# kasvii/GATOR

Measured on AMD Instinct MI355X. Metric: meshes/sec (B=256, J=17) GATOR forward, higher is better.
Workload: dtype f32; 1 GPU; B=256 synthetic Human3.6M 17-joint poses per GPU, GAT+MDR forward fp32; batch_per_gpu=256, global_batch=256, num_joint=17, impl=fused, parallelism=dp1, mode=gather

## Files before the change

### gator_amd/csrc/fused_api.hip

```cpp
#include <hip/hip_runtime.h>

#include <algorithm>
#include <cmath>
#include <cstdlib>
#include <type_traits>
#include <vector>

#include "fused_state.h"
#include "x3_common.h"

namespace gator {
namespace {

static void graph_slot_free(FusedState::GraphSlot& g) {
    if (g.exec) (void)hipGraphExecDestroy((hipGraphExec_t)g.exec);
    if (g.graph) (void)hipGraphDestroy((hipGraph_t)g.graph);
    g.exec = g.graph = nullptr;
}
static void graphs_clear(FusedState* f) {
    for (auto& g : f->graphs) graph_slot_free(g);
    f->graphs.clear();
}
struct WsScope {
    FusedState* f; FusedWs* prev;
    WsScope(FusedState* f_, int i) : f(f_), prev(f_->ws) { f->ws = &f->sets[i]; }
    ~WsScope() { f->ws = prev; }
};

int fused_ensure_ws(gator_ctx* c, int B) {
    FusedState* f = c->fused;
    FusedWs& w = *f->ws;
    if (w.base && B <= w.cap) return GATOR_OK;
    if (w.base) {
        GATOR_HIP_CHECK(hipDeviceSynchronize());
        graphs_clear(f);
    }
    const int cap = B, MT = (cap + 31) / 32, J = c->J;
    const size_t tiles = (size_t)cap * kVT * 2 * kTile;
    size_t n = 0;
    auto layout = [&](float* block) {
        n = 0;
        auto region = [&](auto*& member, size_t floats) {
            if (block) member = reinterpret_cast<std::remove_reference_t<decltype(member)>>(block + n);
            n += (floats + 63) & ~(size_t)63;
        };
        region(w.vcp, (size_t)MT * 3 * kCB * kTile); region(w.vc, (size_t)cap * kV * 3);
        region(w.vf, 3 * tiles); region(w.q, 9 * tiles / 2); region(w.k, 9 * tiles / 2); region(w.v, 9 * tiles / 2);
        region(w.jkv, (size_t)cap * 12 * kTile); region(w.hf, (size_t)cap * kV * 32); region(w.lbf, (size_t)cap * kV * kE);
        region(w.feat, (size_t)cap * J * kC); region(w.vcp3, std::max(upsample_x3_vcp_elems(cap), upsample_x2_vcp_elems(cap)) / 2);
        region(w.lpart, gat_tail_part_floats(cap, J)); region(w.mdr_ctr, mdr_ctr_words(cap)); region(w.hpart, (size_t)cap * kVT * 128);
    };
    layout(nullptr);
    GATOR_TRY(w.base.alloc(n * sizeof(float)));
    GATOR_HIP_CHECK(hipMemset(w.base, 0, n * sizeof(float)));
    GATOR_HIP_CHECK(hipDeviceSynchronize());
    w.cap = cap;
    layout(w.base);
    return GATOR_OK;
}

std::vector<float> d2h(const float* p, size_t n) {
    std::vector<float> v(n);
    (void)hipMemcpy(v.data(), p, n * sizeof(float), hipMemcpyDeviceToHost);
    return v;
}

template <class F>
void fill_tile(float* dst, F tab) {
    for (int g = 0; g < 4; ++g)
        for (int lane = 0; lane < 64; ++lane)
            for (int j = 0; j < 4; ++j) dst[(g * 64 + lane) * 4 + j] = tab(lane & 31, 8 * g + 4 * (lane >> 5) + j);
}

int read_fused_options(const gator_ctx* c, FusedOptions* o) {
    auto flag = [](const char* name, bool dflt) { const char* e = getenv(name); return e ? atoi(e) != 0 : dflt; };
    auto num = [](const char* name, int dflt) { const char* e = getenv(name); return e ? atoi(e) : dflt; };
    auto set = [](const char* name) { return getenv(name) != nullptr; };
    const bool exact = c->arithmetic == GATOR_ARITH_EXACT_SPLIT;
    o->gat_x3 = flag("GATOR_GAT_X3", true);
    o->gat8 = o->gat_x3 && flag("GATOR_GAT8", true);
    o->gat8_h4 = !exact && flag("GATOR_GAT8_H4", true);
    o->gat8_lobyte = o->gat8 && o->gat8_h4 && flag("GATOR_GAT8_LOBYTE", true);
    o->gat_tiled_h4 = !exact && flag("GATOR_GAT_TILED_H4", true);
    o->gat_tiled = num("GATOR_GAT_TILED", -1);
    if (const int m = num("GATOR_GAT_TILED_MIN_BATCH", 0); m > 0) o->gat_tiled_min_batch = m;
    o->mdr_x3 = exact ? 1 : num("GATOR_MDR_X3", 2);
    o->up_x3 = exact ? 1 : num("GATOR_UPSAMPLE_X3", 2);
    if (c->parts & GATOR_PART_MDR) {
        if (o->up_x3 < 0 || o->up_x3 > 2) return fail(GATOR_EINVAL, "GATOR_UPSAMPLE_X3 must be 0, 1 or 2");
        if (o->mdr_x3 < 0 || o->mdr_x3 > 2) return fail(GATOR_EINVAL, "GATOR_MDR_X3 must be 0, 1 or 2");
    }
    o->gat8_tail = o->gat8 && o->gat8_h4 && o->mdr_x3 == 2 && flag("GATOR_GAT8_TAIL", true);
    o->mdr_persist = set("GATOR_MDR_PERSIST") ? flag("GATOR_MDR_PERSIST", false) : -1;
    o->mdr_persist_chunk = num("GATOR_MDR_PERSIST_CHUNK", 0);
    o->mdr_persist_grid = num("GATOR_MDR_PERSIST_GRID", 0);
    o->mdr_head_partials = flag("GATOR_MDR_HEAD_PARTIALS", true);
    o->c3_mdr = o->mdr_x3 == 2 && flag("GATOR_C3_MDR", true);
    o->c3_encoder = o->gat8 && o->gat8_h4 && o->gat_tiled_h4 && flag("GATOR_C3_ENCODER", true);
    o->c3_up_w1 = flag("GATOR_C3_UPSAMPLE_W1", true);
    o->c3_up_bf16 = o->up_x3 != 2 || flag("GATOR_C3_UPSAMPLE_BF16", false);
    o->c3_guard = flag("GATOR_C3_GUARD", true);
    o->graph = flag("GATOR_GRAPH", false);
    o->subbatch_streams = num("GATOR_SUBBATCH_STREAMS", 0);
#ifdef GATOR_DIAG
    o->gat8_dbg = num("GATOR_GAT8_DBG", 0);
    o->gat_stamps = set("GATOR_GAT_STAMPS");
    o->mdr_cut = num("GATOR_MDR_CUT", 0);
    o->mdr_stamps = set("GATOR_MDR_STAMPS");
    o->mdr_solo = set("GATOR_MDR_SOLO");
    o->mdr_ends = set("GATOR_MDR_ENDS");
#endif
    return GATOR_OK;
}

static double sym_eig_max(std::vector<double>& A, int n) {
    for (int sweep = 0; sweep < 64; ++sweep) {
        double off = 0, all = 0;
        for (int p = 0; p < n; ++p)
            for (int q = 0; q < n; ++q) { all += A[p * n + q] * A[p * n + q]; if (q > p) off += A[p * n + q] * A[p * n + q]; }
        if (!(off > 1e-30 * all)) break;
        for (int p = 0; p < n; ++p)
            for (int q = p + 1; q < n; ++q) {
                const double apq = A[p * n + q];
                if (apq == 0) continue;
                const double th = (A[q * n + q] - A[p * n + p]) / (2 * apq);
                const double t = (th >= 0 ? 1.0 : -1.0) / (std::fabs(th) + std::sqrt(th * th + 1));
                const double cs = 1 / std::sqrt(t * t + 1), sn = t * cs;
                for (int k = 0; k < n; ++k) {
                    const double kp = A[k * n + p], kq = A[k * n + q];
                    A[k * n + p] = cs * kp - sn * kq; A[k * n + q] = sn * kp + cs * kq;
                }
                for (int k = 0; k < n; ++k) {
                    const double pk = A[p * n + k], qk = A[q * n + k];
                    A[p * n + k] = cs * pk - sn * qk; A[q * n + k] = sn * pk + cs * qk;
                }
            }
    }
    double m = 0;
    for (int i = 0; i < n; ++i) m = std::max(m, A[i * n + i]);
    return m;
}

float c3_logit_bound(const Weights& w) {
    double worst = 0;
    for (int li = 0; li < 3; ++li) {
        const MdrLayerW& r = w.lay[li];
        const std::vector<float> wq = d2h(r.sa_w[0], 64 * 64), wk = d2h(r.sa_w[1], 64 * 64), bq = d2h(r.sa_b[0], 64), bk = d2h(r.sa_b[1], 64),
                                 a2 = d2h(r.a2, 64), b2 = d2h(r.b2, 64);
        double amax = 0, bn = 0;
        for (int i = 0; i < 64; ++i) { amax = std::max(amax, (double)std::fabs(a2[i])); bn += (double)b2[i] * b2[i]; }
        const double xn = amax * std::sqrt(63.0) + std::sqrt(bn);
        auto head_norm = [&](const std::vector<float>& W, const std::vector<float>& bias, int hd) {
            std::vector<double> G(32 * 32);
            double bb = 0;
            for (int i = 0; i < 32; ++i) {
                bb += (double)bias[32 * hd + i] * bias[32 * hd + i];
                for (int j = 0; j < 32; ++j) {
                    double acc = 0;
                    for (int k = 0; k < 64; ++k) acc += (double)W[(32 * hd + i) * 64 + k] * (double)W[(32 * hd + j) * 64 + k];
                    G[i * 32 + j] = acc;
                }
            }
            return std::sqrt(std::max(sym_eig_max(G, 32), 0.0)) * xn + std::sqrt(bb);
        };
        for (int hd = 0; hd < 2; ++hd)
            worst = std::max(worst, head_norm(wq, bq, hd) * head_norm(wk, bk, hd) / std::sqrt(32.0) * 1.4426950408889634);
    }
    return (float)worst;
}

struct PackItem { const float* src; int64_t wsn, wsk; int N, K; const float** dst; };
template <size_t n>
int pack_linears(const PackItem (&items)[n], float*& p, void* stream) {
    for (const PackItem& it : items) {
        GATOR_TRY(fused_pack_linear(it.src, it.wsn, it.wsk, it.N, it.K, p, stream));
        *it.dst = p;
        p += (size_t)nblk32(it.N) * nblk32(it.K) * kTile;
    }
    return GATOR_OK;
}

int fused_create_gat(gator_ctx* c, FusedState* f, void* stream) {
    const Weights& w = c->w;
    const int J = c->J;
    const size_t blk_tiles = 48 + 16 + 16 + 16 + 16 + 4 + 20 + 64 + 64 + 4 + 4 + 1 + 1;
    const size_t total = (kDepth * blk_tiles + 8 + 2 + 8 + 4 + 12) * kTile;
    GATOR_TRY(f->gbuf.alloc(total * sizeof(float)));
    float* p = f->gbuf;
    auto take = [&](size_t tiles) { float* r = p; p += tiles * kTile; return r; };
    std::vector<float> host;
    auto upload = [&](const std::vector<float>& v) -> const float* {
        float* d = take(v.size() / kTile);
        (void)hipMemcpy(d, v.data(), v.size() * sizeof(float), hipMemcpyHostToDevice);
        return d;
    };
    const std::vector<float> adiag = d2h(c->adj_diag, (size_t)kDepth * J), aoff = d2h(c->adj_off, (size_t)kDepth * J * J),
                             m1 = d2h(c->mask1, (size_t)J * J), m2 = d2h(c->mask2, (size_t)J * J), hb = d2h(c->hop_bias, (size_t)kH * J * J);
    for (int i = 0; i < kDepth; ++i) {
        const GatBlockW& r = w.blk[i];
        GatBlockPk& q = f->gblk[i];
        const PackItem items[] = {
            {r.qkv_w, 128, 1, 384, 128, &q.qkv}, {r.proj_w, 128, 1, 128, 128, &q.proj},
            {r.gcn_W, 1, 128, 128, 128, &q.w0}, {r.gcn_W + 128 * 128, 1, 128, 128, 128, &q.w1},
            {r.xl0_w, 128, 1, 128, 128, &q.lin0}, {r.xl1_w, 128, 1, 16, 128, &q.lin1}, {r.xlb_w, 144, 1, 128, 144, &q.back},
            {r.fc1_w, 128, 1, 512, 128, &q.fc1}, {r.fc2_w, 512, 1, 128, 512, &q.fc2}};
        GATOR_TRY(pack_linears(items, p, stream));
        const std::vector<float> M = d2h(r.gcn_M, (size_t)J * kC), b1 = d2h(r.xl1_b, 16);
        std::vector<float> mc(4 * kTile), md(4 * kTile);
        for (int nb = 0; nb < 4; ++nb) {
            for (int g = 0; g < 4; ++g)
                for (int lane = 0; lane < 64; ++lane)
                    for (int j = 0; j < 4; ++j) {
                        const int tok = 8 * g + 4 * (lane >> 5) + j, n = 32 * nb + (lane & 31);
                        mc[((nb * 4 + g) * 64 + lane) * 4 + j] = tok < J ? M[(size_t)tok * kC + n] : 0.f;
                    }
            fill_tile(md.data() + (size_t)nb * kTile, [&](int t, int ch) { return t < J ? adiag[i * J + t] * M[(size_t)t * kC + 32 * nb + ch] : 0.f; });
        }
        q.mc = upload(mc);
        q.mdT = upload(md);
        std::vector<float> t1(kTile), t2(kTile);
        fill_tile(t1.data(), [&](int t, int j) { return (t < J && j < J) ? aoff[((size_t)i * J + t) * J + j] : 0.f; });
        q.aoffT = upload(t1);
        fill_tile(t2.data(), [&](int t, int ch) {
            if (t >= J || ch >= 16) return 0.f;
            float deg = 0.f;
            for (int j = 0; j < J; ++j) deg += m2[(size_t)t * J + j];
            return deg * b1[ch];
        });
        q.f1b = upload(t2);
    }
    if (f->opt.gat_x3) {
        const int64_t ntiles = (p - f->gblk[0].qkv) / kTile;
        GATOR_TRY(f->gxbuf.alloc((size_t)ntiles * kTileX3 * sizeof(float)));
        int rc = fused_repack_x3(f->gblk[0].qkv, f->gxbuf, ntiles, stream);
        if (rc) return rc;
        if (f->opt.gat_tiled_h4) {
            float left = 0.f;
            GATOR_TRY(f->gxbuf_h3.alloc((size_t)ntiles * kTileX3 * sizeof(float)));
            rc = fused_repack_h3(f->gblk[0].qkv, f->gxbuf_h3, ntiles, &f->gat_tiled_wshift, &left, stream, (int64_t)blk_tiles, 264);
            if (rc == GATOR_OK && left > 1e-7f) rc = fail(GATOR_EUNSUPPORTED, "GAT weights span more than fp16 x 3 planes hold exactly: use GATOR_GAT_TILED_H4=0");
            if (rc) return rc;
        }
        if (f->opt.gat8) {
            rc = gat8_build_stream(f, stream);
            if (rc) return rc;
        }
    }
    std::vector<float> bt(8 * kTile), mt(kTile);
    for (int hd = 0; hd < kH; ++hd)
        fill_tile(bt.data() + (size_t)hd * kTile, [&](int t, int j) { return (t < J && j < J) ? hb[((size_t)hd * J + t) * J + j] : 0.f; });
    f->g_biasT = upload(bt);
    fill_tile(mt.data(), [&](int t, int j) { return (t < J && j < J) ? m1[(size_t)t * J + j] : 0.f; });
    f->g_m1T = upload(mt);
    fill_tile(mt.data(), [&](int t, int j) { return (t < J && j < J) ? m2[(size_t)t * J + j] : 0.f; });
    f->g_m2T = upload(mt);
    {
        std::vector<float> vv((size_t)kDepth * 2048);
        for (int i = 0; i < kDepth; ++i) {
            const GatBlockW& r = w.blk[i];
            const struct { const float* p; int n; } parts[] = {{r.n1w, 128}, {r.n1b, 128}, {r.qkv_b, 384}, {r.proj_b, 128}, {r.gcn_bias, 128},
                                                               {r.xl0_b, 128}, {r.xlb_b, 128}, {r.n2w, 128}, {r.n2b, 128}, {r.fc1_b, 512}, {r.fc2_b, 128}};
            size_t off = (size_t)i * 2048;
            for (auto& pt : parts) {
                const std::vector<float> h = d2h(pt.p, pt.n);
                std::copy(h.begin(), h.end(), vv.begin() + off);
                off += pt.n;
            }
        }
        f->g_vecs = upload(vv);
    }
    {
        float* dst = take(8);
        int rc = fused_pack_linear(w.gl3_W, 64, 1, 128, 64, dst, stream);
        if (rc) return rc;
        f->g_gl3 = dst;
        const std::vector<float> pe = d2h(c->pos_embed, (size_t)J * kC);
        std::vector<float> pt(4 * kTile);
        for (int kb = 0; kb < 4; ++kb)
            fill_tile(pt.data() + (size_t)kb * kTile, [&](int t, int ch) { return t < J ? pe[(size_t)t * kC + 32 * kb + ch] : 0.f; });
        f->g_posT = upload(pt);
    }
    {
        int rc = gat_prepare_device();
        if (rc == GATOR_OK) rc = gat_tiled_prepare_device();
        if (rc == GATOR_OK) rc = gat8_prepare_device();
        if (rc) return rc;
        hipDeviceProp_t prop;
        if (hipGetDeviceProperties(&prop, c->device) == hipSuccess && prop.multiProcessorCount > 0) f->n_cu = prop.multiProcessorCount;
    }
    GATOR_HIP_CHECK(hipStreamSynchronize((hipStream_t)stream));
    GATOR_HIP_CHECK(hipGetLastError());
    return GATOR_OK;
}

}

int fused_create(gator_ctx* c, void* stream) {
    if (c->impl == GATOR_IMPL_BASIC) return GATOR_OK;
    FusedState* f = new FusedState();
    c->fused = f;
    int rc = read_fused_options(c, &f->opt);
    if (rc) return rc;
    f->gat_tiled = f->opt.gat_tiled;
    f->graph_replay = f->opt.graph;
    const Weights& w = c->w;
    if (c->parts & GATOR_PART_GAT) {
        rc = fused_create_gat(c, f, stream);
        if (rc) return rc;
    }
    if (!(c->parts & GATOR_PART_MDR)) return GATOR_OK;
    if (f->opt.c3_mdr) {
        f->c3_logit_bound = c3_logit_bound(w);
        if (f->opt.c3_guard && !(f->c3_logit_bound <= 1024.0f)) f->opt.c3_mdr = f->opt.c3_encoder = false;
    }
    const size_t n_up = f->opt.up_x3 == 0 ? (size_t)3 * kOB * kCB * kTile : 0, n_layer = (size_t)64 * kTile;
    const size_t total = n_up + 3 * n_layer + 24 * kTile + 64 + (size_t)kVT * 2 * kTile + 3 * 64 + 1024;
    GATOR_TRY(f->wbuf.alloc(total * sizeof(float)));
    float* p = f->wbuf;
    auto take = [&](size_t k) { float* r = p; p += k; return r; };
    float* up = take(n_up);
    if (f->opt.up_x3 == 2) {
        GATOR_TRY(f->up_w2.alloc(upsample_x2_weight_elems() * 2));
        int rc = pack_upsample_x2(w.up_w, f->up_w2, &f->up_w2_unscale, stream);
        if (rc == GATOR_OK) rc = upsample_x2_prepare_device();
        if (rc) return rc;
    } else if (f->opt.up_x3 == 1) {
        GATOR_TRY(f->up_w3.alloc(upsample_x3_weight_elems() * 2));
        int rc = pack_upsample_x3(w.up_w, f->up_w3, stream);
        if (rc) return rc;
    } else {
        for (int tap = 0; tap < 3; ++tap) {
            int rc = fused_pack_linear(w.up_w + tap, (int64_t)kV * 3, 3, kNV, kV, up + (size_t)tap * kOB * kCB * kTile, stream);
            if (rc) return rc;
        }
        f->up_w = up;
    }
    for (int li = 0; li < 3; ++li) {
        const MdrLayerW& r = w.lay[li];
        MdrLayerP& q = f->lay[li];
        const PackItem items[] = {
            {r.wq, 64, 1, 64, 64, &q.wq}, {r.wk, 64, 1, 64, 64, &q.wk}, {r.wv, 64, 1, 64, 64, &q.wv}, {r.proj_w, 64, 1, 64, 64, &q.proj},
            {r.fc1_w, 64, 1, 256, 64, &q.fc1}, {r.fc2_w, 256, 1, 64, 256, &q.fc2},
            {r.sa_w[0], 64, 1, 64, 64, &q.sa[0]}, {r.sa_w[1], 64, 1, 64, 64, &q.sa[1]}, {r.sa_w[2], 64, 1, 64, 64, &q.sa[2]}, {r.sa_w[3], 64, 1, 64, 64, &q.sa[3]}};
        GATOR_TRY(pack_linears(items, p, stream));
    }
    {
        std::vector<float> hw(32 * 64, 0.f), hb(32, 0.f);
        const std::vector<float> mw = d2h(w.motion_w, 23 * 64), mb = d2h(w.motion_b, 23), bw = d2h(w.biasl_w, 3 * 64), bb = d2h(w.biasl_b, 3);
        for (int r = 0; r < 20; ++r) { std::copy(mw.begin() + r * 64, mw.begin() + (r + 1) * 64, hw.begin() + r * 64); hb[r] = mb[r]; }
        for (int r = 0; r < 3; ++r) {
            std::copy(bw.begin() + r * 64, bw.begin() + (r + 1) * 64, hw.begin() + (24 + r) * 64); hb[24 + r] = bb[r];
            std::copy(mw.begin() + (20 + r) * 64, mw.begin() + (21 + r) * 64, hw.begin() + (28 + r) * 64); hb[28 + r] = mb[20 + r];
        }
        if (c->alpha) {
            const std::vector<float> sw = d2h(w.scale_w, 64), sb = d2h(w.scale_b, 1);
            std::copy(sw.begin(), sw.end(), hw.begin() + 27 * 64);
            hb[27] = sb[0];
        }
        DevBuf<float> tmp;
        GATOR_TRY(tmp.alloc(hw.size() * sizeof(float)));
        GATOR_HIP_CHECK(hipMemcpy(tmp, hw.data(), hw.size() * sizeof(float), hipMemcpyHostToDevice));
        float* dst = take(2 * kTile);
        int rc = fused_pack_linear(tmp, 64, 1, 32, 64, dst, stream);
        GATOR_HIP_CHECK(hipStreamSynchronize((hipStream_t)stream));
        tmp.reset();
        if (rc) return rc;
        f->head_w = dst;
        if (f->opt.mdr_x3) {
            const int64_t ntiles = (dst + 2 * kTile - f->lay[0].wq) / kTile;
            GATOR_TRY(f->wxbuf.alloc((size_t)ntiles * kTileX3 * sizeof(float)));
            if (f->opt.mdr_x3 == 2) {
                float left = 0.f;
                rc = fused_repack_h3(f->lay[0].wq, f->wxbuf, ntiles, &f->mdr_wshift, &left, stream);
                if (rc == GATOR_OK && left > 1e-7f) rc = fail(GATOR_EUNSUPPORTED, "MDR weights span more than fp16 x 3 planes hold exactly (residual %.2e of the largest weight): use GATOR_MDR_X3=1", left);
            } else {
                rc = fused_repack_x3(f->lay[0].wq, f->wxbuf, ntiles, stream);
            }
            if (rc) return rc;
        }
        float* hbd = take(64);
        GATOR_HIP_CHECK(hipMemcpy(hbd, hb.data(), 32 * sizeof(float), hipMemcpyHostToDevice));
        f->head_b = hbd;
    }
    {
        float* dst = take(10 * kTile);
        int rc = fused_pack_linear(w.jfeat_w, 133, 1, 64, 133, dst, stream);
        if (rc) return rc;
        f->jfeat_p = dst;
        float* d128 = take(8 * kTile);
        rc = fused_pack_linear(w.jfeat_w + 5, 133, 1, 64, 128, d128, stream);
        if (rc) return rc;
        f->jfeat128_p = d128;
        if (f->opt.mdr_x3 == 2) {
            float left = 0.f;
            GATOR_TRY(f->jf128_h3.alloc((size_t)8 * kTileX3 * sizeof(float)));
// ... 359 lines not shown
```

### gator_amd/csrc/fused_state.h

```cpp
#pragma once
#include "internal.h"
#include <vector>

namespace gator {

constexpr int kVT = 14;
constexpr int kOB = 216;
constexpr int kCB = 14;
constexpr int kTile = 32 * 32;
constexpr int kMdrCtrChunks = 64;
__host__ __device__ inline size_t mdr_ctr_words(int B) { return (size_t)32 * kMdrCtrChunks + (size_t)4 * B; }

struct MdrLayerP {
    const float *wq, *wk, *wv, *proj, *fc1, *fc2, *sa[4];
};

struct GatBlockPk {
    const float *qkv, *proj, *w0, *w1, *lin0, *lin1, *back, *fc1, *fc2;
    const float *mc, *mdT, *aoffT, *f1b;
};

struct FusedWs {
    DevBuf<float> base;
    int cap = 0;
    float *vcp = nullptr;
    void* vcp3 = nullptr;
    float *vc = nullptr;
    float *vf = nullptr, *q = nullptr, *k = nullptr, *v = nullptr;
    float *jkv = nullptr;
    float *hf = nullptr;
    float *lbf = nullptr;
    float *feat = nullptr;
    float* hpart = nullptr;
    float *lpart = nullptr;
    bool mdr_ctr_clean = false;
    unsigned* mdr_ctr = nullptr;
    DevBuf<void> vcp16;
    int vcp16_cap = 0;
};

struct FusedOptions {
    bool gat_x3 = true;
    bool gat8 = true;
    bool gat8_h4 = true;
    bool gat8_lobyte = true;
    bool gat8_tail = true;
    bool gat_tiled_h4 = true;
    int gat_tiled = -1;
    int gat_tiled_min_batch = 1024;
    int mdr_x3 = 2;
    int up_x3 = 2;
    int mdr_persist = -1;
    int mdr_persist_chunk = 0;
    int mdr_persist_grid = 0;
    bool mdr_head_partials = true;
    bool c3_mdr = true;
    bool c3_encoder = true;
    bool c3_up_w1 = true;
    bool c3_up_bf16 = false;
    bool c3_guard = true;
    bool graph = false;
    int subbatch_streams = 0;
    int gat8_dbg = 0;
    bool gat_stamps = false;
    int mdr_cut = 0;
    bool mdr_stamps = false;
    bool mdr_solo = false;
    bool mdr_ends = false;
};

struct FusedState {
    ~FusedState();
    FusedOptions opt;
    DevBuf<float> wbuf;
    DevBuf<float> gbuf;
    GatBlockPk gblk[kDepth];
    const float *g_biasT = nullptr, *g_m1T = nullptr, *g_m2T = nullptr, *g_gl3 = nullptr, *g_posT = nullptr, *g_vecs = nullptr;
    const float* up_w = nullptr;
    DevBuf<void> up_w3;
    int gat_tiled = -1;
    int n_cu = 256;
    DevBuf<float> gxbuf;
    DevBuf<float> gxbuf_h3;
    int gat_tiled_wshift = 0;
    DevBuf<float> g8stream;
    DevBuf<float> g8stream_b;
    int gat8_wshift = 0;
    DevBuf<float> wxbuf;
    DevBuf<float> jf128_h3;
    int jf128_wshift = 0;
    int mdr_wshift = 0;
    float c3_logit_bound = 0.f;
    DevBuf<void> up_w2;
    float up_w2_unscale = 1.f;
    DevBuf<void> up_w16;
    DevBuf<void> jr_blk, jr_ent;
    DevBuf<float> jr_w;
    DevBuf<int> jr_rowptr;
    DevBuf<float> jr_P;
    int jr_nnz = 0, jr_nj = 0, jr_cap = 0;
    DevBuf<float> blk_tap;
    int blk_tap_cap = 0;
    MdrLayerP lay[3];
    const float* head_w = nullptr;
    const float* head_b = nullptr;
    const float* tok_base = nullptr;
    const float* tok_w3 = nullptr;
    struct GraphSlot {
        int B = 0; const void *in = nullptr, *verts = nullptr, *pose3d = nullptr; bool bf16 = false;
        int tiled = 0, persist = 0; const void* ws = nullptr;
        void *graph = nullptr, *exec = nullptr;
        unsigned long long used = 0;
    };
    static constexpr int kGraphSlots = 8;
    bool graph_replay = false;
    void* cap_stream = nullptr;
    std::vector<GraphSlot> graphs;
    unsigned long long graph_clock = 0, graph_launches = 0;
    FusedWs sets[2];
    FusedWs* ws = &sets[0];
    void* aux_stream = nullptr;
    void *ev_fork = nullptr, *ev_join = nullptr;
    const float* jfeat_p = nullptr;
    const float* jfeat5 = nullptr;
    const float* jfeat128_p = nullptr;
    const float* posj_T = nullptr;
};

int fused_pack_linear(const float* W, int64_t wsn, int64_t wsk, int N, int K, float* dst, void* stream);
inline int nblk32(int n) { return (n + 31) / 32; }
int launch_pack_vc(const float* vc, int B, float* vcp, void* stream);
int launch_upsample(const FusedState* f, const gator_ctx* c, int B, float* verts, void* stream);
int gat_prepare_device();
int gat_ensure_blk_tap(gator_ctx* c, FusedState* f, int B);
int launch_gat(gator_ctx* c, FusedState* f, const float* pose2d, int B, float* x_out, float* feat, void* stream, bool split_tail = false,
               int B_total = 0, int tap_row0 = 0, bool half16 = false, float* tail_jkv = nullptr);
int gat8_prepare_device();
int gat8_build_stream(FusedState* f, void* stream);
int launch_gat8(gator_ctx* c, FusedState* f, const float* pose2d, int B, float* feat, void* stream, int B_total = 0, int tap_row0 = 0, bool half16 = false,
                float* tail_x_out = nullptr, float* tail_jkv = nullptr, int ctr_B = 0);
bool gat8_tail_supported(const FusedState* f, bool half16);
int gat_tiled_prepare_device();
int gat_tiled_samples_per_wg(int J);
int launch_gat_tiled(gator_ctx* c, FusedState* f, const float* pose2d, int B, float* feat, void* stream, int B_total = 0, bool half16 = false);
size_t gat_tail_part_floats(int B, int J);
int launch_gat_tail(gator_ctx* c, FusedState* f, const float* pose2d, const float* feat, int B, float* x_out, void* stream, bool zero_ctr = true);
size_t upsample_bf16_weight_elems();
size_t upsample_bf16_vcp_elems(int B);
int pack_upsample_bf16(const float* up_w, void* dst, void* stream);
int launch_upsample_bf16(const FusedState* f, const gator_ctx* c, const float* vc, int B, float* verts, void* stream);
size_t upsample_x3_weight_elems();
size_t upsample_x3_vcp_elems(int B);
int pack_upsample_x3(const float* up_w, void* dst, void* stream);
int launch_pack_vc_x3(const float* vc, int B, int cap, void* vcp3, void* stream);
int launch_upsample_x3(const FusedState* f, const gator_ctx* c, int B, float* verts, void* stream, bool with_joints = false);
int launch_jreg_reduce(const FusedState* f, int B, float* joints, void* stream);
size_t upsample_x2_weight_elems();
size_t upsample_x2_vcp_elems(int B);
int upsample_x2_prepare_device();
int pack_upsample_x2(const float* up_w, void* dst, float* unscale, void* stream);
int launch_pack_vc_x2(const float* vc, int B, void* vcp2, void* stream);
int launch_upsample_x2(const FusedState* f, const gator_ctx* c, int B, float* verts, void* stream, bool with_joints = false, bool w1 = false);
int launch_upsample_any(const FusedState* f, const gator_ctx* c, int B, float* verts, void* stream, bool with_joints = false, bool w1 = false);
int launch_mdr(gator_ctx* c, FusedState* f, const float* pc, int B, void* stream, const float* x_out = nullptr, const float* pose2d = nullptr, bool half16 = false);

}
```

### gator_amd/csrc/upsample_x2.hip

```cpp
#include <cmath>
#include <cstring>

#include "upsample_common.h"

namespace gator {
namespace {

constexpr int kNBuf = 4, kStageFrags = 36;
constexpr int kActShift = 4;

__device__ __forceinline__ void split2(float x, _Float16& h, _Float16& l) {
    h = (_Float16)x;
    l = (_Float16)(x - (float)h);
}

__global__ void k_pack_up_x2(const float* __restrict__ w, _Float16* __restrict__ dst, int64_t n_frag_pairs, float scale) {
    const int64_t e = (int64_t)blockIdx.x * blockDim.x + threadIdx.x;
    if (e >= n_frag_pairs * 512) return;
    const int j = e & 7, lane = (e >> 3) & 63;
    int64_t r = e >> 9;
    const int tap = r % 3; r /= 3;
    const int o2 = r & 1; r >>= 1;
    const int s = r % kS16;
    const int op = (int)(r / kS16);
    const int o = 32 * (2 * op + o2) + (lane & 31), c = 16 * s + 8 * (lane >> 5) + j;
    const float x = (o < kNV && c < kV) ? w[((int64_t)o * kV + c) * 3 + tap] * scale : 0.f;
    _Float16 h, l;
    split2(x, h, l);
    const int64_t pair = (((int64_t)op * kS16 + s) * 2 + o2) * 3 + tap;
    dst[(pair * 2 + 0) * 512 + lane * 8 + j] = h;
    dst[(pair * 2 + 1) * 512 + lane * 8 + j] = l;
}
__global__ void k_pack_vc_x2(const float* __restrict__ vc, int B, _Float16* __restrict__ ap, int64_t n_frag_pairs) {
    const int64_t e = (int64_t)blockIdx.x * blockDim.x + threadIdx.x;
    if (e >= n_frag_pairs * 512) return;
    const int j = e & 7, lane = (e >> 3) & 63;
    int64_t r = e >> 9;
    const int lp = r % 3; r /= 3;
    const int mi = r & 3; r >>= 2;
    const int s = r % kS16;
    const int mg = (int)(r / kS16);
    const int smp = 32 * (4 * mg + mi) + (lane & 31), c = 16 * s + 8 * (lane >> 5) + j;
    const float x = (smp < B && c < kV) ? vc[((int64_t)smp * kV + c) * 3 + lp] * (float)(1 << kActShift) : 0.f;
    _Float16 h, l;
    split2(x, h, l);
    const int64_t pair = (((int64_t)mg * kS16 + s) * 4 + mi) * 3 + lp;
    ap[(pair * 2 + 0) * 512 + lane * 8 + j] = h;
    ap[(pair * 2 + 1) * 512 + lane * 8 + j] = l;
}

__global__ void k_absmax(const float* __restrict__ w, int64_t n, unsigned* __restrict__ out) {
    float m = 0.f;
    for (int64_t i = (int64_t)blockIdx.x * blockDim.x + threadIdx.x; i < n; i += (int64_t)gridDim.x * blockDim.x) {
        const float a = fabsf(w[i]);
        m = a > m || a != a ? a : m;
    }
    for (int o = 32; o > 0; o >>= 1) {
        const float q = __shfl_xor(m, o);
        m = q > m || q != q ? q : m;
    }
    if ((threadIdx.x & 63) == 0) atomicMax(out, __float_as_uint(m));
}

__device__ __forceinline__ void dma_frag(const void* base, unsigned lane_off, unsigned lds_dst) {
    unsigned keep;
    asm volatile("s_mov_b32 %0, m0\n\ts_mov_b32 m0, %3\n\ts_nop 0\n\tglobal_load_lds_dwordx4 %1, %2\n\ts_mov_b32 m0, %0"
                 : "=&s"(keep) : "v"(lane_off), "s"(base), "s"(lds_dst) : "memory");
}
template <int N> __device__ __forceinline__ void wait_vm() { asm volatile("s_waitcnt vmcnt(%0)" ::"n"(N) : "memory"); }

template <bool WLO = true>
__global__ __launch_bounds__(512, 1) void k_upsample_x2(const _Float16* __restrict__ ap, const _Float16* __restrict__ wp,
                                                        const float* __restrict__ bias, const float* __restrict__ tpl,
                                                        float* __restrict__ out, int B, int MT, int MG, int nwg, float unscale,
                                                        const JregEpi jr) {
    extern __shared__ __attribute__((aligned(16))) unsigned char lds_raw[];
    f16x8 (*st)[kStageFrags][64] = reinterpret_cast<f16x8 (*)[kStageFrags][64]>(lds_raw);
    const int lane = threadIdx.x & 63, wave = __builtin_amdgcn_readfirstlane(threadIdx.x >> 6);
    const int wg = xcd_remap(blockIdx.x, nwg);
    const int obp = wg / MG, mg = wg % MG;
    const int mi = wave & 3, oi = wave >> 2;
    const int ob = 2 * obp + oi, mt = 4 * mg + mi;
    const bool live = mt < MT;
    const unsigned lane_off = lane * 16;
    const unsigned lds0 = (unsigned)(unsigned long long)lds_raw;
    const char* a_src = reinterpret_cast<const char*>(ap) + (size_t)mg * kS16 * 24 * 1024;
    const char* w_src = reinterpret_cast<const char*>(wp) + (size_t)obp * kS16 * 12 * 1024;
    const char* src[5];
    unsigned stride[5], dsto[5];
#pragma unroll
    for (int i = 0; i < 5; ++i) {
        const int f = wave + 8 * i;
        src[i] = f < 24 ? a_src + f * 1024 : w_src + (f - 24) * 1024;
        stride[i] = f < 24 ? 24 * 1024 : 12 * 1024;
        dsto[i] = lds0 + f * 1024;
    }
    auto issue = [&](int s) {
        const unsigned dst = (unsigned)(s & (kNBuf - 1)) * kStageFrags * 1024;
#pragma unroll
        for (int i = 0; i < 4; ++i) dma_frag(src[i] + (size_t)s * stride[i], lane_off, dst + dsto[i]);
        if (wave < 4) dma_frag(src[4] + (size_t)s * stride[4], lane_off, dst + dsto[4]);
    };
    auto wait_landed = [&](int younger) {
        if (younger >= 1) { if (wave < 4) wait_vm<5>(); else wait_vm<4>(); }
        else wait_vm<0>();
    };
    f32x16 big[3], sm[3], tot[3];
#pragma unroll
    for (int l = 0; l < 3; ++l) { big[l] = zero16(); sm[l] = zero16(); tot[l] = zero16(); }
    f16x8 a[3][2], w[3][2];
    auto load_first = [&](int s) {
        const f16x8 (*cur)[64] = st[s & (kNBuf - 1)];
#pragma unroll
        for (int p = 0; p < 2; ++p) {
            a[0][p] = cur[mi * 6 + p][lane];
            w[0][p] = cur[24 + oi * 6 + p][lane];
            w[1][p] = cur[24 + oi * 6 + 2 + p][lane];
        }
    };
    auto load_rest = [&](int s) {
        const f16x8 (*cur)[64] = st[s & (kNBuf - 1)];
#pragma unroll
        for (int p = 0; p < 2; ++p) {
            a[1][p] = cur[mi * 6 + 2 + p][lane];
            w[2][p] = cur[24 + oi * 6 + 4 + p][lane];
            a[2][p] = cur[mi * 6 + 4 + p][lane];
        }
    };
    issue(0); issue(1); issue(2);
    if (wave < 4) wait_vm<10>(); else wait_vm<8>();
    __builtin_amdgcn_s_barrier();
    load_first(0);
#pragma unroll 1
    for (int s = 0; s < kS16; ++s) {
        if (s + 1 < kS16) wait_landed(kS16 - 2 - s);
        __builtin_amdgcn_s_barrier();
        if (s + 3 < kS16) issue(s + 3);
        load_rest(s);
        if (live) {
#pragma unroll
            for (int lp = 0; lp < 3; ++lp)
#pragma unroll
                for (int k = 2; k >= 0; --k) {
                    const int l = lp + 1 - k;
                    if (l < 0 || l > 2) continue;
                    big[l] = GATOR_MFMA_F16(a[lp][0], w[k][0], big[l]);
                    if constexpr (WLO) sm[l] = GATOR_MFMA_F16(a[lp][0], w[k][1], sm[l]);
                    sm[l] = GATOR_MFMA_F16(a[lp][1], w[k][0], sm[l]);
                }
            if (s % 7 == 6) {
#pragma unroll
                for (int l = 0; l < 3; ++l) { tot[l] += big[l]; big[l] = zero16(); }
            }
        }
        if (s + 1 < kS16) load_first(s + 1);
    }
    const int ov = 32 * ob + (lane & 31), h = lane >> 5;
    if (ov >= kNV || !live) return;
    const float bo = bias[ov];
    const float t0 = tpl[ov * 3], t1 = tpl[ov * 3 + 1], t2 = tpl[ov * 3 + 2];
    const int2 jb = jr.P ? jr.blk[ob] : int2{0, 0};
#pragma unroll
    for (int r = 0; r < 16; ++r) {
        const int smp = 32 * mt + kap(r) + 4 * h;
        if (smp < B) {
            F3 v;
            v.x = ((tot[0][r] + sm[0][r]) * unscale + bo) + t0;
            v.y = ((tot[1][r] + sm[1][r]) * unscale + bo) + t1;
            v.z = ((tot[2][r] + sm[2][r]) * unscale + bo) + t2;
            if (out) *reinterpret_cast<F3*>(out + ((int64_t)smp * kNV + ov) * 3) = v;
            for (int e = jb.x; e < jb.x + jb.y; ++e) {
                const int2 en = jr.ent[e];
                if (en.x == ov) {
                    const float we = jr.w[e];
                    F3 q;
                    q.x = we * v.x; q.y = we * v.y; q.z = we * v.z;
                    *reinterpret_cast<F3*>(jr.P + ((int64_t)smp * jr.nnz + en.y) * 3) = q;
                }
            }
        }
    }
}

constexpr size_t kX2Lds = (size_t)kNBuf * kStageFrags * 1024;

}

size_t upsample_x2_weight_elems() { return (size_t)(kOB / 2) * kS16 * 12 * 512; }
size_t upsample_x2_vcp_elems(int B) { return (size_t)((B + 127) / 128) * kS16 * 24 * 512; }

int upsample_x2_prepare_device() {
    GATOR_HIP_CHECK(hipFuncSetAttribute((const void*)k_upsample_x2<true>, hipFuncAttributeMaxDynamicSharedMemorySize, (int)kX2Lds));
    GATOR_HIP_CHECK(hipFuncSetAttribute((const void*)k_upsample_x2<false>, hipFuncAttributeMaxDynamicSharedMemorySize, (int)kX2Lds));
    return GATOR_OK;
}

int pack_upsample_x2(const float* up_w, void* dst, float* unscale, void* stream) {
    hipStream_t st = (hipStream_t)stream;
    DevBuf<unsigned> d_max;
    GATOR_TRY(d_max.alloc(sizeof(unsigned)));
    GATOR_HIP_CHECK(hipMemsetAsync(d_max, 0, sizeof(unsigned), st));
    const int64_t n = (int64_t)kNV * kV * 3;
    k_absmax<<<1024, 256, 0, st>>>(up_w, n, d_max.get());
    unsigned bits = 0;
    GATOR_HIP_CHECK(hipMemcpyAsync(&bits, d_max, sizeof(unsigned), hipMemcpyDeviceToHost, st));
    GATOR_HIP_CHECK(hipStreamSynchronize(st));
    d_max.reset();
    float wmax;
    static_assert(sizeof(wmax) == sizeof(bits), "float bits");
    memcpy(&wmax, &bits, sizeof(wmax));
    int shift = 0;
    if (wmax > 0.f && std::isfinite(wmax)) {
        int e;
        (void)std::frexp(wmax, &e);
        shift = 14 - e;
        if (shift > 118) shift = 118;
        if (shift < -118) shift = -118;
    }
    const int64_t pairs = (int64_t)upsample_x2_weight_elems() / 1024;
    k_pack_up_x2<<<(unsigned)((pairs * 512 + 255) / 256), 256, 0, st>>>(up_w, (_Float16*)dst, pairs, std::ldexp(1.0f, shift));
    GATOR_HIP_CHECK(hipGetLastError());
    *unscale = std::ldexp(1.0f, -(shift + kActShift));
    return GATOR_OK;
}

int launch_pack_vc_x2(const float* vc, int B, void* vcp2, void* stream) {
    const int64_t pairs = (int64_t)upsample_x2_vcp_elems(B) / 1024;
    k_pack_vc_x2<<<(unsigned)((pairs * 512 + 255) / 256), 256, 0, (hipStream_t)stream>>>(vc, B, (_Float16*)vcp2, pairs);
    GATOR_HIP_CHECK(hipGetLastError());
    return GATOR_OK;
}

int launch_upsample_x2(const FusedState* f, const gator_ctx* c, int B, float* verts, void* stream, bool with_joints, bool w1) {
    const int MT = (B + 31) / 32, MG = (MT + 3) / 4;
    const JregEpi jr = jreg_epi(f, with_joints);
    const int nwg = (kOB / 2) * MG;
    if (w1) k_upsample_x2<false><<<nwg, 512, kX2Lds, (hipStream_t)stream>>>((const _Float16*)f->ws->vcp3, (const _Float16*)f->up_w2.get(), c->w.up_b, c->w.v6890,
                                                                           verts, B, MT, MG, nwg, f->up_w2_unscale, jr);
    else k_upsample_x2<true><<<nwg, 512, kX2Lds, (hipStream_t)stream>>>((const _Float16*)f->ws->vcp3, (const _Float16*)f->up_w2.get(), c->w.up_b, c->w.v6890,
                                                                       verts, B, MT, MG, nwg, f->up_w2_unscale, jr);
    GATOR_HIP_CHECK(hipGetLastError());
    return GATOR_OK;
}

}
```

Baseline: 436,000 meshes/sec.

## Make upsample_x2 kernel persistent with cross-tile prefetch of next tile's stages

Turns the upsample_x2 MFMA kernel into a persistent kernel: the grid is capped at the CU count (or an override) and each workgroup loops over tiles. While finishing the current tile it issues the DMA for the next tile's first stages, so loads overlap the epilogue and launch/prologue cost is paid once per workgroup. It also prefetches bias/template values two steps early and splits the epilogue into separate output and joint-regressor loops. The risks are more template variants, higher register pressure from the live next-tile state, and a tail imbalance when the tile count does not divide evenly across the grid.

Result: no change. 437,500 meshes/sec, median of 4 (+0.3%).

```diff
diff --git a/gator_amd/csrc/fused_api.hip b/gator_amd/csrc/fused_api.hip
--- a/gator_amd/csrc/fused_api.hip
+++ b/gator_amd/csrc/fused_api.hip
@@ -91,6 +91,8 @@
         if (o->mdr_x3 < 0 || o->mdr_x3 > 2) return fail(GATOR_EINVAL, "GATOR_MDR_X3 must be 0, 1 or 2");
     }
     o->gat8_tail = o->gat8 && o->gat8_h4 && o->mdr_x3 == 2 && flag("GATOR_GAT8_TAIL", true);
+    o->up_persist = flag("GATOR_UPSAMPLE_PERSIST", true);
+    o->up_grid = num("GATOR_UPSAMPLE_GRID", 0);
     o->mdr_persist = set("GATOR_MDR_PERSIST") ? flag("GATOR_MDR_PERSIST", false) : -1;
     o->mdr_persist_chunk = num("GATOR_MDR_PERSIST_CHUNK", 0);
     o->mdr_persist_grid = num("GATOR_MDR_PERSIST_GRID", 0);
diff --git a/gator_amd/csrc/fused_state.h b/gator_amd/csrc/fused_state.h
--- a/gator_amd/csrc/fused_state.h
+++ b/gator_amd/csrc/fused_state.h
@@ -50,6 +50,8 @@
     int gat_tiled_min_batch = 1024;
     int mdr_x3 = 2;
     int up_x3 = 2;
+    bool up_persist = true;
+    int up_grid = 0;
     int mdr_persist = -1;
     int mdr_persist_chunk = 0;
     int mdr_persist_grid = 0;
diff --git a/gator_amd/csrc/upsample_x2.hip b/gator_amd/csrc/upsample_x2.hip
--- a/gator_amd/csrc/upsample_x2.hip
+++ b/gator_amd/csrc/upsample_x2.hip
@@ -8,6 +8,7 @@
 
 constexpr int kNBuf = 4, kStageFrags = 36;
 constexpr int kActShift = 4;
+constexpr int kSteps = (kV + 15) / 16;
 
 __device__ __forceinline__ void split2(float x, _Float16& h, _Float16& l) {
     h = (_Float16)x;
@@ -69,7 +70,7 @@
 }
 template <int N> __device__ __forceinline__ void wait_vm() { asm volatile("s_waitcnt vmcnt(%0)" ::"n"(N) : "memory"); }
 
-template <bool WLO = true>
+template <bool WLO = true, bool PERSIST = true>
 __global__ __launch_bounds__(512, 1) void k_upsample_x2(const _Float16* __restrict__ ap, const _Float16* __restrict__ wp,
                                                         const float* __restrict__ bias, const float* __restrict__ tpl,
                                                         float* __restrict__ out, int B, int MT, int MG, int nwg, float unscale,
@@ -77,40 +78,31 @@
     extern __shared__ __attribute__((aligned(16))) unsigned char lds_raw[];
     f16x8 (*st)[kStageFrags][64] = reinterpret_cast<f16x8 (*)[kStageFrags][64]>(lds_raw);
     const int lane = threadIdx.x & 63, wave = __builtin_amdgcn_readfirstlane(threadIdx.x >> 6);
-    const int wg = xcd_remap(blockIdx.x, nwg);
-    const int obp = wg / MG, mg = wg % MG;
     const int mi = wave & 3, oi = wave >> 2;
-    const int ob = 2 * obp + oi, mt = 4 * mg + mi;
-    const bool live = mt < MT;
     const unsigned lane_off = lane * 16;
     const unsigned lds0 = (unsigned)(unsigned long long)lds_raw;
-    const char* a_src = reinterpret_cast<const char*>(ap) + (size_t)mg * kS16 * 24 * 1024;
-    const char* w_src = reinterpret_cast<const char*>(wp) + (size_t)obp * kS16 * 12 * 1024;
-    const char* src[5];
-    unsigned stride[5], dsto[5];
-#pragma unroll
-    for (int i = 0; i < 5; ++i) {
-        const int f = wave + 8 * i;
-        src[i] = f < 24 ? a_src + f * 1024 : w_src + (f - 24) * 1024;
-        stride[i] = f < 24 ? 24 * 1024 : 12 * 1024;
-        dsto[i] = lds0 + f * 1024;
-    }
-    auto issue = [&](int s) {
-        const unsigned dst = (unsigned)(s & (kNBuf - 1)) * kStageFrags * 1024;
-#pragma unroll
-        for (int i = 0; i < 4; ++i) dma_frag(src[i] + (size_t)s * stride[i], lane_off, dst + dsto[i]);
-        if (wave < 4) dma_frag(src[4] + (size_t)s * stride[4], lane_off, dst + dsto[4]);
+    struct Src { const char *a, *w; };
+    auto tile_src = [&](int wg) {
+        return Src{reinterpret_cast<const char*>(ap) + ((size_t)(wg % MG) * kS16 * 24 + wave) * 1024,
+                   reinterpret_cast<const char*>(wp) + ((size_t)(wg / MG) * kS16 * 12 + wave) * 1024};
+    };
+    auto issue = [&](const Src& p, int s, unsigned slot) {
+        const unsigned dst = lds0 + ((slot & (kNBuf - 1)) * kStageFrags + wave) * 1024;
+        const char* a_s = p.a + (size_t)s * (24 * 1024);
+        const char* w_s = p.w + (size_t)s * (12 * 1024);
+#pragma unroll
+        for (int i = 0; i < 3; ++i) dma_frag(a_s + i * 8192, lane_off, dst + i * 8192);
+        dma_frag(w_s, lane_off, dst + 24 * 1024);
+        if (wave < 4) dma_frag(w_s + 8192, lane_off, dst + 32 * 1024);
     };
     auto wait_landed = [&](int younger) {
         if (younger >= 1) { if (wave < 4) wait_vm<5>(); else wait_vm<4>(); }
         else wait_vm<0>();
     };
     f32x16 big[3], sm[3], tot[3];
-#pragma unroll
-    for (int l = 0; l < 3; ++l) { big[l] = zero16(); sm[l] = zero16(); tot[l] = zero16(); }
     f16x8 a[3][2], w[3][2];
-    auto load_first = [&](int s) {
-        const f16x8 (*cur)[64] = st[s & (kNBuf - 1)];
+    auto load_first = [&](unsigned slot) {
+        const f16x8 (*cur)[64] = st[slot & (kNBuf - 1)];
 #pragma unroll
         for (int p = 0; p < 2; ++p) {
             a[0][p] = cur[mi * 6 + p][lane];
@@ -118,8 +110,8 @@
             w[1][p] = cur[24 + oi * 6 + 2 + p][lane];
         }
     };
-    auto load_rest = [&](int s) {
-        const f16x8 (*cur)[64] = st[s & (kNBuf - 1)];
+    auto load_rest = [&](unsigned slot) {
+        const f16x8 (*cur)[64] = st[slot & (kNBuf - 1)];
 #pragma unroll
         for (int p = 0; p < 2; ++p) {
             a[1][p] = cur[mi * 6 + 2 + p][lane];
@@ -127,58 +119,94 @@
             a[2][p] = cur[mi * 6 + 4 + p][lane];
         }
     };
-    issue(0); issue(1); issue(2);
+    float bo = 0.f, t0 = 0.f, t1 = 0.f, t2 = 0.f;
+    int t = blockIdx.x, wg = xcd_remap(t, nwg);
+    unsigned g = 0;
+    Src src = tile_src(wg), nsrc = src;
+    issue(src, 0, 0); issue(src, 1, 1); issue(src, 2, 2);
     if (wave < 4) wait_vm<10>(); else wait_vm<8>();
     __builtin_amdgcn_s_barrier();
     load_first(0);
+    for (;;) {
+        const int tn = t + (int)gridDim.x;
+        const bool more = PERSIST && tn < nwg;
+        const int wgn = more ? xcd_remap(tn, nwg) : 0;
+        if (more) nsrc = tile_src(wgn);
+        const int ob = 2 * (wg / MG) + oi, mt = 4 * (wg % MG) + mi;
+        const bool live = mt < MT;
+        const int ov = 32 * ob + (lane & 31), h = lane >> 5;
+#pragma unroll
+        for (int l = 0; l < 3; ++l) { big[l] = zero16(); sm[l] = zero16(); tot[l] = zero16(); }
 #pragma unroll 1
-    for (int s = 0; s < kS16; ++s) {
-        if (s + 1 < kS16) wait_landed(kS16 - 2 - s);
-        __builtin_amdgcn_s_barrier();
-        if (s + 3 < kS16) issue(s + 3);
-        load_rest(s);
-        if (live) {
-#pragma unroll
-            for (int lp = 0; lp < 3; ++lp)
-#pragma unroll
-                for (int k = 2; k >= 0; --k) {
-                    const int l = lp + 1 - k;
-                    if (l < 0 || l > 2) continue;
-                    big[l] = GATOR_MFMA_F16(a[lp][0], w[k][0], big[l]);
-                    if constexpr (WLO) sm[l] = GATOR_MFMA_F16(a[lp][0], w[k][1], sm[l]);
-                    sm[l] = GATOR_MFMA_F16(a[lp][1], w[k][0], sm[l]);
+        for (int s = 0; s < kSteps; ++s) {
+            if (more) wait_landed(1);
+            else if (s + 1 < kSteps) wait_landed(kSteps - 2 - s);
+            __builtin_amdgcn_s_barrier();
+            if (s == kSteps - 2 && ov < kNV) {
+                bo = bias[ov];
+                t0 = tpl[ov * 3]; t1 = tpl[ov * 3 + 1]; t2 = tpl[ov * 3 + 2];
+            }
+            if (s + 3 < kSteps) issue(src, s + 3, g + s + 3);
+            else if (more) issue(nsrc, s + 3 - kSteps, g + s + 3);
+            load_rest(g + s);
+            if (live) {
+#pragma unroll
+                for (int lp = 0; lp < 3; ++lp)
+#pragma unroll
+                    for (int k = 2; k >= 0; --k) {
+                        const int l = lp + 1 - k;
+                        if (l < 0 || l > 2) continue;
+                        big[l] = GATOR_MFMA_F16(a[lp][0], w[k][0], big[l]);
+                        if constexpr (WLO) sm[l] = GATOR_MFMA_F16(a[lp][0], w[k][1], sm[l]);
+                        sm[l] = GATOR_MFMA_F16(a[lp][1], w[k][0], sm[l]);
+                    }
+                if (s % 7 == 6) {
+#pragma unroll
+                    for (int l = 0; l < 3; ++l) { tot[l] += big[l]; big[l] = zero16(); }
                 }
-            if (s % 7 == 6) {
-#pragma unroll
-                for (int l = 0; l < 3; ++l) { tot[l] += big[l]; big[l] = zero16(); }
-            }
-        }
-        if (s + 1 < kS16) load_first(s + 1);
-    }
-    const int ov = 32 * ob + (lane & 31), h = lane >> 5;
-    if (ov >= kNV || !live) return;
-    const float bo = bias[ov];
-    const float t0 = tpl[ov * 3], t1 = tpl[ov * 3 + 1], t2 = tpl[ov * 3 + 2];
-    const int2 jb = jr.P ? jr.blk[ob] : int2{0, 0};
-#pragma unroll
-    for (int r = 0; r < 16; ++r) {
-        const int smp = 32 * mt + kap(r) + 4 * h;
-        if (smp < B) {
-            F3 v;
-            v.x = ((tot[0][r] + sm[0][r]) * unscale + bo) + t0;
-            v.y = ((tot[1][r] + sm[1][r]) * unscale + bo) + t1;
-            v.z = ((tot[2][r] + sm[2][r]) * unscale + bo) + t2;
-            if (out) *reinterpret_cast<F3*>(out + ((int64_t)smp * kNV + ov) * 3) = v;
-            for (int e = jb.x; e < jb.x + jb.y; ++e) {
-                const int2 en = jr.ent[e];
-                if (en.x == ov) {
-                    const float we = jr.w[e];
-                    F3 q;
-                    q.x = we * v.x; q.y = we * v.y; q.z = we * v.z;
-                    *reinterpret_cast<F3*>(jr.P + ((int64_t)smp * jr.nnz + en.y) * 3) = q;
+            }
+            if (more || s + 1 < kSteps) load_first(g + s + 1);
+        }
+        if (live && ov < kNV) {
+#pragma unroll
+            for (int l = 0; l < 3; ++l) tot[l] += big[l];
+            auto vertex = [&](int r) {
+                F3 v;
+                v.x = ((tot[0][r] + sm[0][r]) * unscale + bo) + t0;
+                v.y = ((tot[1][r] + sm[1][r]) * unscale + bo) + t1;
+                v.z = ((tot[2][r] + sm[2][r]) * unscale + bo) + t2;
+                return v;
+            };
+            asm volatile("" :: "v"(bo), "v"(t0), "v"(t1), "v"(t2));
+            if (out) {
+#pragma unroll
+                for (int r = 0; r < 16; ++r) {
+                    const int smp = 32 * mt + kap(r) + 4 * h;
+                    if (smp < B) *reinterpret_cast<F3*>(out + ((int64_t)smp * kNV + ov) * 3) = vertex(r);
                 }
             }
-        }
+            if (jr.P) {
+                const int2 jb = jr.blk[ob];
+#pragma unroll
+                for (int r = 0; r < 16; ++r) {
+                    const int smp = 32 * mt + kap(r) + 4 * h;
+                    if (smp < B) {
+                        const F3 v = vertex(r);
+                        for (int e = jb.x; e < jb.x + jb.y; ++e) {
+                            const int2 en = jr.ent[e];
+                            if (en.x == ov) {
+                                const float we = jr.w[e];
+                                F3 q;
+                                q.x = we * v.x; q.y = we * v.y; q.z = we * v.z;
+                                *reinterpret_cast<F3*>(jr.P + ((int64_t)smp * jr.nnz + en.y) * 3) = q;
+                            }
+                        }
+                    }
+                }
+            }
+        }
+        if (!more) break;
+        t = tn; wg = wgn; g += kSteps; src = nsrc;
     }
 }
 
@@ -189,9 +217,16 @@
 size_t upsample_x2_weight_elems() { return (size_t)(kOB / 2) * kS16 * 12 * 512; }
 size_t upsample_x2_vcp_elems(int B) { return (size_t)((B + 127) / 128) * kS16 * 24 * 512; }
 
+template <bool WLO, bool PERSIST>
+static int x2_allow_lds() {
+    GATOR_HIP_CHECK(hipFuncSetAttribute((const void*)k_upsample_x2<WLO, PERSIST>, hipFuncAttributeMaxDynamicSharedMemorySize, (int)kX2Lds));
+    return GATOR_OK;
+}
 int upsample_x2_prepare_device() {
-    GATOR_HIP_CHECK(hipFuncSetAttribute((const void*)k_upsample_x2<true>, hipFuncAttributeMaxDynamicSharedMemorySize, (int)kX2Lds));
-    GATOR_HIP_CHECK(hipFuncSetAttribute((const void*)k_upsample_x2<false>, hipFuncAttributeMaxDynamicSharedMemorySize, (int)kX2Lds));
+    GATOR_TRY((x2_allow_lds<true, true>()));
+    GATOR_TRY((x2_allow_lds<true, false>()));
+    GATOR_TRY((x2_allow_lds<false, true>()));
+    GATOR_TRY((x2_allow_lds<false, false>()));
     return GATOR_OK;
 }
 
@@ -231,14 +266,26 @@
     return GATOR_OK;
 }
 
+template <bool WLO, bool PERSIST>
+static void x2_launch(int grid, hipStream_t st, const FusedState* f, const gator_ctx* c, float* verts, int B, int MT, int MG, int nwg, const JregEpi& jr) {
+    k_upsample_x2<WLO, PERSIST><<<grid, 512, kX2Lds, st>>>((const _Float16*)f->ws->vcp3, (const _Float16*)f->up_w2.get(), c->w.up_b, c->w.v6890,
+                                                         verts, B, MT, MG, nwg, f->up_w2_unscale, jr);
+}
+
 int launch_upsample_x2(const FusedState* f, const gator_ctx* c, int B, float* verts, void* stream, bool with_joints, bool w1) {
     const int MT = (B + 31) / 32, MG = (MT + 3) / 4;
     const JregEpi jr = jreg_epi(f, with_joints);
     const int nwg = (kOB / 2) * MG;
-    if (w1) k_upsample_x2<false><<<nwg, 512, kX2Lds, (hipStream_t)stream>>>((const _Float16*)f->ws->vcp3, (const _Float16*)f->up_w2.get(), c->w.up_b, c->w.v6890,
-                                                                           verts, B, MT, MG, nwg, f->up_w2_unscale, jr);
-    else k_upsample_x2<true><<<nwg, 512, kX2Lds, (hipStream_t)stream>>>((const _Float16*)f->ws->vcp3, (const _Float16*)f->up_w2.get(), c->w.up_b, c->w.v6890,
-                                                                       verts, B, MT, MG, nwg, f->up_w2_unscale, jr);
+    hipStream_t st = (hipStream_t)stream;
+    if (f->opt.up_persist) {
+        const int want = f->opt.up_grid > 0 ? f->opt.up_grid : f->n_cu;
+        const int grid = want < nwg ? want : nwg;
+        if (w1) x2_launch<false, true>(grid, st, f, c, verts, B, MT, MG, nwg, jr);
+        else x2_launch<true, true>(grid, st, f, c, verts, B, MT, MG, nwg, jr);
+    } else {
+        if (w1) x2_launch<false, false>(nwg, st, f, c, verts, B, MT, MG, nwg, jr);
+        else x2_launch<true, false>(nwg, st, f, c, verts, B, MT, MG, nwg, jr);
+    }
     GATOR_HIP_CHECK(hipGetLastError());
     return GATOR_OK;
 }
```
